# volser/FluidFramework

Measured on AMD Instinct MI355X. Metric: sequenced merge-tree ops applied/sec (whole node) + achieved HBM GB/s, higher is better.
Workload: dtype int32; 1 GPU; config2: 4096 docs x 8 clients x 10k msgs, lag U[0,32], 60/40 ins/rem; docs_per_gpu=4096, msgs_per_doc=10000, clients=8, lag_max=32, parallelism=doc-sharded x1, residency=blk, big_min_ops=0

## Files before the change

fluidframework_amd/csrc/mt_core.h:

```cpp
#pragma once
#include <type_traits>
#include "wave.h"
#include "../../include/mtgpu.h"

#define MT_MAXH 16
#define MT_PSK 16
#define MT_PKEYS MT_MAX_PROP_KEYS
#define MT_MAXN 8
#define MT_GRAN 256
#define MT_ZMAX 2
#define MT_NOREM 0x7FFFFFFF
#define MT_RFL 128
#ifndef MT_L_ROWS
#define MT_L_ROWS 256
#endif
#ifndef MT_L_BLKS
#define MT_L_BLKS 96
#endif
#ifndef MT_L_HEAP
#define MT_L_HEAP 96
#endif
#define MT_L_H 8
#ifndef MT_B_BLKS
#define MT_B_BLKS 104
// ... 220 lines not shown
#define MT_DREC_SLACK (2 + 2 * 2 * (8 + 64))

struct __attribute__((aligned(16))) MtLoadSeg {
    uint8_t flags, pad0; uint16_t client;
    int32_t seq, rseq;
    uint16_t rclient; int16_t prop;
    uint32_t poff, plen;
    uint32_t mid, pad1;
};
enum { MT_LD_START = 0, MT_LD_CONT = 1, MT_LD_REFLUSH = 2, MT_LD_REFLUSH_NEW = 3, MT_LD_UNSUPPORTED = 4 };
struct MtLoadStep { int seg, kind, cli, seq; };
struct MtLoad {
    const uint32_t* docs; const uint32_t* seg_off; const uint32_t* nhdr;
    const int32_t* ms; const int32_t* cs;
    const MtLoadSeg* segs; const uint16_t* payload;
    const uint32_t* plan_off; const MtLoadStep* plan;
};
#define MT_NONCOLLAB 0xFFFE
#define MT_NOBODY 0xFFFF

struct MtGen {
    unsigned long long seed;
    uint32_t ops, clients, lag_max, pct_insert, pct_remove, ins_len_max, rem_len_max, n_ann_sets, pct_rewrite;
    int enabled;
    const uint32_t* clients_per_run;
    uint32_t doc_id_base;
    uint32_t ins_len_min, seg_prop_sets, ins_at_end;
    uint64_t total_ops;
};

struct __attribute__((aligned(16))) MtQ16 { uint32_t x, y, z, w; };
struct __attribute__((aligned(16))) MtLdsPools {
    MtRow rows[MT_L_ROWS];
    MtBlk blk[MT_L_BLKS];
    MtHeapE heap[MT_L_HEAP + 2];
    int win[MT_L_ROWS];
    int uid[MT_L_ROWS];
    int udelta[MT_L_ROWS];
    uint8_t uanc[MT_L_ROWS * MT_L_H];
};

template <int NB, int NH, int NT, int NW> struct __attribute__((aligned(16))) MtLdsBlkT {
    static_assert(NB <= NT, "block ids index the corrections table");
    MtBlk blk[NB];
    MtHeapE heap[NH + 2];
    int win[NW];
    int bcorr[NT];
};
using MtLdsBlk = MtLdsBlkT<MT_B_BLKS, MT_B_HEAP, MT_B_BT, MT_B_W>;
using MtLdsBlkW = MtLdsBlkT<MT_BW_BLKS, MT_BW_HEAP, MT_BW_BT, MT_BW_W>;

struct __attribute__((aligned(16))) MtLdsBig {
    MtHeapE heap[MT_G_HEAP + 2];
    int win[MT_G_WIN];
    int uid[MT_G_U], udelta[MT_G_U];
    int uanc[MT_G_U * MT_G_H];
    uint16_t ulist[MT_G_U];
    MtBlk spare0; int spare1;
    int sid[MT_G_STG], sdel[MT_G_STG], spf[MT_G_STG];
    int htk[MT_G_HT], htv[MT_G_HT];
    uint16_t hlist[MT_G_HT];
    uint32_t bpc[MT_G_BP];
    struct Job {
        int op, r, c, r0, n, H, minSeq, heapN;
        MtRow* R; int* win; MtBlk* blk; int* uanc; uint16_t* text;
    } mw[2];
    int posted;
};

struct MtScratch {
    int pathB[MT_MAXH + 2], pathJ[MT_MAXH + 2];
    int pathOff[MT_MAXH + 2], pathLen[MT_MAXH + 2];
    int hold[64];
    int holdLen[64];
    uint8_t holdBlk[64];
    int rfree[MT_RFL];
    int corr[MT_MAXN];
};

struct __attribute__((aligned(16), may_alias)) MtQ16a { uint32_t x, y, z, w; };
#ifndef MT_RANGE_LEAF
#define MT_RANGE_LEAF 1
#endif
#ifndef MT_GT_CH
#define MT_GT_CH 4
#endif
MT_INLINE int pick16(const int* c, int j) {
    int v = c[0];
#pragma unroll
    for (int i = 1; i < 16; i++) v = (j == i) ? c[i] : v;
    return v;
}
MT_INLINE int pick8(const int* c, int j) {
    int v = c[0];
#pragma unroll
    for (int i = 1; i < 8; i++) v = (j == i) ? c[i] : v;
    return v;
}
MT_INLINE bool ovl_has(const MtOvx* ox, int n, unsigned long long ovl, int s, int rseq, int c) {
    if (c < 63) return ((ovl >> c) & 1ull) != 0;
    const bool more = (ovl >> 63) != 0;
    bool f = false;
    for (int i = 0; i < n; i++) {
        const MtOvx e = ox[i];
        f = f | (more & (e.row == s) & (e.client == c) & (e.rseq == rseq));
    }
    return f;
}
MT_INLINE bool vis_rc(int seq, uint32_t meta, int rseq, uint32_t rcl, unsigned long long ovl, int r, int c,
                      const MtOvx* ox, int nox, int s) {
    const int cl = (int)(meta & MT_M_CLIENT);
    const bool seen = (cl == c) | (seq <= r);
    const bool removed = (meta & MT_M_REMOVED) != 0;
    const bool gone = ((int)rcl == c) | (rseq <= r) | ovl_has(ox, nox, ovl, s, rseq, c);
    return seen & !(removed & gone);
}

struct BlkH { int len, parent, n, height, scour; };
struct ChildL { int len; bool tie; };
struct WinI { int id; int delta; int parent; bool live; bool recycle; };

enum { MT_WALK_SPLIT = 0, MT_WALK_INSERT = 1, MT_WALK_RANGE = 2 };
enum { MT_W_OK = 0, MT_W_NOCHANGE = 1, MT_W_FAIL = 2, MT_W_RANGED = 3 };
enum { MT_MAP_REMOVE = 0, MT_MAP_ANNOTATE = 1, MT_MAP_COLLECT = 2 };
enum { MT_PM_SET = 0, MT_PM_REWRITE = 1, MT_PM_INCR = 2, MT_PM_KEEP = 3, MT_PM_CONS = 4, MT_PM_INCR_SMIN = 5 };
MT_INLINE int mt_prop_mode(uint32_t fl) {
    if (!(fl & MT_OPF_COMBINE)) return (fl & MT_OPF_REWRITE) ? MT_PM_REWRITE : MT_PM_SET;
    if (fl & MT_OPF_REWRITE) return (fl & MT_OPF_CONSENSUS) ? MT_PM_CONS : MT_PM_KEEP;
    return (fl & MT_OPF_INCR_STRMIN) ? MT_PM_INCR_SMIN : MT_PM_INCR;
}

struct MtEngParams {
    uint32_t rowCap, heapCap, winCap, textCap, psetCap, p_nsets;
    uint16_t* textBase;
    const uint32_t* p_off; const uint16_t* p_key; const int32_t* p_val;
    const uint8_t* p_falsy; const uint32_t* p_class; const int32_t* p_vinfo;
};
#if defined(__HIP_DEVICE_COMPILE__)
#define MT_LDS_VAR(T, v) __shared__ T v
#else
#define MT_LDS_VAR(T, v) static T v
#endif
MT_LDS_VAR(MtLdsPools, mt_lds_pools_v);
MT_INLINE MtLdsPools& mt_lds() { return mt_lds_pools_v; }
MT_LDS_VAR(MtLdsBlk, mt_ldsb_v);
MT_INLINE MtLdsBlk& mt_ldsb() { return mt_ldsb_v; }
MT_LDS_VAR(MtLdsBlkW, mt_ldsbw_v);
MT_INLINE MtLdsBlkW& mt_ldsbw() { return mt_ldsbw_v; }
MT_LDS_VAR(MtLdsBig, mt_ldsg_v);
MT_INLINE MtLdsBig& mt_ldsg() { return mt_ldsg_v; }

struct MtCold {
    MtEngParams S;
    uint32_t cnt[6];
    int hw[2];
    int lcap[3];
    uint32_t gcap[4];
    int epoch, ncol, midcap;
    uint32_t op;
    MtDocHdr* hdr; int* rfhbm; MtOvx* ovx; int* midt; MtReg* regs;
    MtBlk* blk; MtHeapE* heap; int *uid, *udelta, *uanc; MtPSet* pset;
    int ovxn, blkfreen, texthalf, psettop;
    uint16_t* dtext; unsigned long long dtcap;
    uint32_t dused, tused; int dstop;
    int* regr; int regTop, regHalf, regCap;
    int pcKey[4], pcVal[4];
// ... 31 lines not shown
    MT_HD MtBlk& bk(int b) const {
        if constexpr (LDS) return mt_lds().blk[b]; else if constexpr (BLKL) return LB().blk[b];
        else return blk[b];
    }
    MT_HD MtHeapE& hp(int k) const {
        if constexpr (LDS) return mt_lds().heap[k]; else if constexpr (BLKL) return LB().heap[k];
        else if constexpr (BIG) return mt_ldsg().heap[k]; else return heap[k];
    }
    static constexpr int kW = BW ? MT_BW_W : MT_B_W;
    MT_HD int winGet(int k) const {
        if constexpr (BLKR) { if (k < kW) return LB().win[k]; return win[k]; }
        else return wn(k);
    }
    MT_HD void winSet(int k, int v) const {
        if constexpr (BLKR) { if (k < kW) LB().win[k] = v; else win[k] = v; }
        else wn(k) = v;
    }
    MT_HD int& wn(int k) const {
        static_assert(!BLKR, "block residency: winGet / winSet");
        if constexpr (LDS) return mt_lds().win[k];
        else if constexpr (BIG) { if (k < lRows) return mt_ldsg().win[k]; return win[k]; }
        else return win[k];
    }
    MT_HD int& ui(int k) const { if constexpr (LDS) return mt_lds().uid[k]; else return uid[k]; }
    MT_HD int& ud(int k) const { if constexpr (LDS) return mt_lds().udelta[k]; else return udelta[k]; }
    static constexpr bool UL = RES == MT_RES_BIG;
    static constexpr bool BT = BLKR;
    static constexpr int UCAP = RES == MT_RES_BIG ? MT_G_U : 0;
    template <bool L> MT_HD int uiAt(int k) const {
        if constexpr (UL && L) return mt_ldsg().uid[k];
        else return ui(k);
    }
    template <bool L> MT_HD int udAt(int k) const {
        if constexpr (UL && L) return mt_ldsg().udelta[k];
        else return ud(k);
    }
    template <bool L> MT_HD void uPutAt(int k, int id, int delta) {
        if constexpr (UL && L) { mt_ldsg().uid[k] = id; mt_ldsg().udelta[k] = delta; }
        else { ui(k) = id; ud(k) = delta; }
    }
    template <bool L> MT_HD void ancPutAt(int u, int h, int a) {
        if constexpr (UL && L) {
            static_assert(BIG, "block residency keeps per-block corrections, not ancestor chains");
            mt_ldsg().uanc[u * MT_G_H + h] = a;
        } else ancPut(u, h, a);
    }
    template <bool L> MT_HD int ancGetAt(int u, int h) const {
        if constexpr (UL && L) {
            static_assert(BIG, "block residency keeps per-block corrections, not ancestor chains");
            return mt_ldsg().uanc[u * MT_G_H + h];
        } else return ancGet(u, h);
    }
    MT_HD void ancPutAny(int u, int h, int a) {
        if constexpr (UL) { if (u < UCAP) ancPutAt<true>(u, h, a); else ancPutAt<false>(u, h, a); }
        else ancPut(u, h, a);
    }
    MT_HD int ancGetAny(int u, int h) const {
        if constexpr (UL) { if (u < UCAP) return ancGetAt<true>(u, h); return ancGetAt<false>(u, h); }
        else return ancGet(u, h);
    }
    template <class F> MT_HD void forU(F f) const {
        for (int base = 0; base < nU; base += MT_WAVE) {
            const int m = (nU - base) < MT_WAVE ? (nU - base) : MT_WAVE;
            if (UL && base < UCAP) f(std::true_type{}, base, m);
            else f(std::false_type{}, base, m);
        }
    }
    int root, height, minSeq, curSeq, rowTop, blkTop, blkFree, heapN, winN, textTop;
    int& psetTop = mt_cold_v.psettop;
    uint32_t status;
    uint32_t &c_ops = mt_cold_v.cnt[0], &c_msgs = mt_cold_v.cnt[1], &c_ins = mt_cold_v.cnt[2], &c_rows = mt_cold_v.cnt[3],
             &c_depth = mt_cold_v.cnt[4], &c_scour = mt_cold_v.cnt[5];
    unsigned long long prof[8];
    int& textHalf = mt_cold_v.texthalf; uint32_t blkCap;
    int nU; bool uValid; int uRef, uCli;
    int heapTop;
    int& gcEpoch = mt_cold_v.epoch;
    int lastL, lastIdx; bool lastSplit;
    bool htOk; int hlistN;
    bool htOn, pfOn; int mwSeq;
    bool bpOn;
    int& nCol = mt_cold_v.ncol;
    int landB;
    int rfN; int*& rfHbm = mt_cold_v.rfhbm;
    int& blkFreeN = mt_cold_v.blkfreen;
    int &heapHW = mt_cold_v.hw[0], &winHW = mt_cold_v.hw[1];
    static constexpr bool kLds = BLKL || BIG;
    int &lRows = mt_cold_v.lcap[0], &lBlks = mt_cold_v.lcap[1], &lHeap = mt_cold_v.lcap[2];
    uint32_t &gRowCap = mt_cold_v.gcap[0], &gBlkCap = mt_cold_v.gcap[1], &gHeapCap = mt_cold_v.gcap[2],
             &gWinCap = mt_cold_v.gcap[3];

    MT_HD void bind(const MtState& st, uint32_t d, MtScratch* scratch) {
        const MtDocLayout* Ly = st.layout + d;
        auto off = [&](const unsigned long long* p) -> size_t {
            const uint32_t* w = (const uint32_t*)p;
            return (size_t)uni(w[0]) | ((size_t)uni(w[1]) << 32);
        };
        S.rowCap = uni(Ly->rowCap); S.heapCap = uni(Ly->heapCap); S.winCap = uni(Ly->winCap); S.textCap = uni(Ly->textCap);
        S.psetCap = uni(Ly->psetCap); S.p_nsets = st.p_nsets; S.p_off = st.p_off; S.p_key = st.p_key; S.p_val = st.p_val;
        S.p_falsy = st.p_falsy; S.p_class = st.p_class; S.p_vinfo = st.p_vinfo; S.textBase = st.text + off(&Ly->text);
        blkCap = uni(Ly->blkCap); hdrp = st.hdr + d;
        R = st.rows + off(&Ly->row);
        blk = st.blk + off(&Ly->blk); heap = st.heap + off(&Ly->heap);
        const size_t wo = off(&Ly->win);
        win = st.win + wo; uid = st.uid + wo; udelta = st.udelta + wo; uanc = st.uanc + off(&Ly->anc);
        pset = st.pset + off(&Ly->pset);
        ovx = st.ovx + (size_t)d * MT_OVX_CAP;
        regs = st.reg + (size_t)d * MT_REG_CAP;
        regr = st.regr + off(&Ly->regr); regCap = (int)uni(Ly->regCap);
        midt = st.mid + off(&Ly->mid); midCap = (int)uni(Ly->midCap);
        drec = nullptr; dcount = nullptr; dcap = 0; curOp = 0;
        dtext = nullptr; dtcap = 0; dUsed = 0; tUsed = 0; dStop = 0;
        sc = scratch;
        const MtDocHdr& h = *hdrp;
        root = uni(h.root); height = uni(h.height); minSeq = uni(h.minSeq); curSeq = uni(h.curSeq); rowTop = uni(h.rowTop);
        blkTop = uni(h.blkTop); blkFree = uni(h.blkFree); heapN = uni(h.heapN); winN = uni(h.winN); textTop = uni(h.textTop);
        psetTop = uni(h.psetTop); status = uni(h.status); textHalf = uni(h.textHalf);
        text = S.textBase + (size_t)textHalf * S.textCap;
#if MT_KEEP_PROF
        for (int i = 0; i < 8; i++) prof[i] = h.prof[i];
#endif
        c_ops = c_msgs = c_ins = c_rows = c_depth = c_scour = 0;
        nU = 0; uValid = false; uRef = -1; uCli = -1;
        heapTop = heapN > 0 ? uni(heap[1].maxSeq) : 0x7FFFFFFF;
        lastL = 0; lastIdx = 0; lastSplit = false; gcEpoch = 0; htOk = false; hlistN = 0; htOn = pfOn = false; mwSeq = 0; bpOn = false;
        for (int i = 0; i < 4; i++) mt_cold_v.pcKey[i] = -1;
        rfHbm = st.hold + (size_t)d * MT_RFL; rfN = uni(h.rfN); blkFreeN = uni(h.blkFreeN);
        heapHW = uni(h.heapHW); winHW = uni(h.winHW); ovxN = uni(h.ovxN);
        regTop = uni(h.regTop); regHalf = uni(h.regHalf) & 1; mt_cold_v.pNever = uni(h.pNever);
        if (regTop < 0 || regTop > regCap) regTop = 0;
        if (ovxN < 0 || ovxN > MT_OVX_CAP) ovxN = 0;
        lRows = lBlks = lHeap = 0; gRowCap = gBlkCap = gHeapCap = gWinCap = 0;
        if (rfN < 0 || rfN > MT_RFL) rfN = 0;
        { const int n = rfN; const int* src = rfHbm;
          for (int base = 0; base < n; base += MT_WAVE) {
              const int m = (n - base) < MT_WAVE ? (n - base) : MT_WAVE;
              wave_for(m, [&](int k) MT_LAM { sc->rfree[base + k] = src[base + k]; });
          } }
        wave_sync();
    }
    MT_HD void store(uint32_t) {
        MtDocHdr& h = *hdrp;
        h.root = root; h.height = height; h.minSeq = minSeq; h.curSeq = curSeq; h.rowTop = rowTop;
        h.blkTop = blkTop; h.blkFree = blkFree; h.heapN = heapN; h.winN = winN; h.textTop = textTop;
        h.psetTop = psetTop; h.status = status; h.textHalf = textHalf; h.rfN = rfN; h.blkFreeN = blkFreeN;
        h.heapHW = heapHW; h.winHW = winHW; h.ovxN = ovxN; h.regTop = regTop; h.regHalf = regHalf;
        h.pNever = mt_cold_v.pNever;
        { const int n = rfN; int* dst = rfHbm;
          for (int base = 0; base < n; base += MT_WAVE) {
              const int m = (n - base) < MT_WAVE ? (n - base) : MT_WAVE;
              wave_for(m, [&](int k) MT_LAM { dst[base + k] = sc->rfree[base + k]; });
          } }
#if MT_KEEP_PROF
        for (int i = 0; i < 8; i++) h.prof[i] = prof[i];
#endif
        h.cnt[0] += c_ops; h.cnt[1] += c_msgs; h.cnt[2] += c_ins; h.cnt[3] += c_rows; h.cnt[4] += c_depth;
        h.cnt[5] += c_scour;
    }
    MT_HD void open() {
        root = 0; height = 0; minSeq = 0; curSeq = 0; rowTop = 0; blkTop = 1; blkFree = -1;
        heapN = 0; winN = 0; textTop = 0; psetTop = 0; status = 0; textHalf = 0; heapTop = 0x7FFFFFFF; rfN = 0;
        for (int i = 0; i < 4; i++) mt_cold_v.pcKey[i] = -1;
        blkFreeN = 0; heapHW = 0; winHW = 0; ovxN = 0;
        text = S.textBase;
        c_ops = c_msgs = c_ins = c_rows = c_depth = c_scour = 0;
        for (int i = 0; i < 6; i++) hdrp->cnt[i] = 0;
        for (int i = 0; i < 8; i++) prof[i] = 0;
#if !MT_KEEP_PROF
        for (int i = 0; i < 8; i++) hdrp->prof[i] = 0;
#endif
        wave_for(8, [&](int i) MT_LAM { bk(0).c[i] = -1; });
        bk(0).len = 0; bk(0).parent = -1; bk(0).n = 0; bk(0).height = 0; bk(0).scour = -1;
        bpReset();
        wave_for(MT_REG_CAP, [&](int i) MT_LAM { regs[i].client = -1; regs[i].n = 0; regs[i].flags = 0; regs[i].off = 0; });
        regTop = 0; regHalf = 0; mt_cold_v.pNever = 0;
    }

    MT_HD int allocRow() {
        if (rfN > 0) { rfN--; return uni(sc->rfree[rfN]); }
        if (rowTop >= (int)S.rowCap) { status |= MT_DS_OOM_ROWS; return -1; }
        return rowTop++;
    }
    MT_HD void freeRow(int s) { if (rfN < MT_RFL) { sc->rfree[rfN] = s; rfN++; } }
    MT_HD int allocBlock() {
        if (blkFree >= 0) { const int id = blkFree; blkFree = uni(bk(id).parent); blkFreeN--; return id; }
        if (blkTop >= (int)blkCap) { status |= MT_DS_OOM_BLOCKS; return -1; }
        return blkTop++;
    }
    MT_HD void freeBlock(int id) { bk(id).parent = blkFree; bk(id).n = -1; blkFree = id; blkFreeN++; bpDrop(id); }
    MT_HD static uint32_t bpPack(int b, int p) { return ((uint32_t)(b >> MT_G_BPL) << 20) | (uint32_t)(p + 1); }
    MT_HD void bpPut(int b, int p) {
        if constexpr (BIG) {
            if (bpOn) {
                uint32_t& e = mt_ldsg().bpc[b & (MT_G_BP - 1)];
                if (e != MT_BP_EMPTY && (e >> 20) != (uint32_t)(b >> MT_G_BPL)) MT_BS(4);
                e = bpPack(b, p);
            }
        }
    }
    MT_HD void bpDrop(int b) {
        if constexpr (BIG) {
            if (bpOn) {
                uint32_t& e = mt_ldsg().bpc[b & (MT_G_BP - 1)];
                if ((e >> 20) == (uint32_t)(b >> MT_G_BPL)) MT_BS(5);
                e = MT_BP_EMPTY;
            }
        }
    }
// ... 886 lines not shown
        int w = 0;
        for (int base = 0; base < n0; base += MT_WAVE) {
            const int m = (n0 - base) < MT_WAVE ? (n0 - base) : MT_WAVE;
            auto u = wave_map(m, [&](int k) MT_LAM { return lsN < 0 ? base + k : (int)mt_ldsg().ulist[base + k]; });
            auto keep = wave_map(m, [&](int k) MT_LAM { return mt_ldsg().uanc[own(u, k) * MT_G_H + hc] == child; });
            const auto rk = wave_rank(keep);
            const int cnt = wave_count(keep), w0 = w;
            wave_sync();
            wave_for(m, [&](int k) MT_LAM { if (own(keep, k)) mt_ldsg().ulist[w0 + own(rk, k)] = (uint16_t)own(u, k); });
            w += cnt;
        }
        wave_sync();
        return w;
    }

    MT_HD void ovxCompact() {
        int w = 0;
        for (int base = 0; base < ovxN; base += MT_WAVE) {
            const int m = (ovxN - base) < MT_WAVE ? (ovxN - base) : MT_WAVE;
            auto keep = wave_map(m, [&](int k) MT_LAM {
                const MtOvx e = ovx[base + k];
                return (bool)((int)(row(e.row).parent >= 0) & (int)(row(e.row).rseq == e.rseq) & (int)(e.rseq > minSeq));
            });
            auto ent = wave_map(m, [&](int k) MT_LAM { return ovx[base + k]; });
            auto rk = wave_rank(keep);
            const int cnt = wave_count(keep);
            wave_sync();
            const int w0 = w;
            wave_for(m, [&](int k) MT_LAM { if (own(keep, k)) ovx[w0 + own(rk, k)] = own(ent, k); });
            wave_sync();
            w += cnt;
        }
        ovxN = w;
    }
    MT_HD void ovxAdd(int s, int rseq, int c) {
        if (ovxN >= MT_OVX_CAP) ovxCompact();
        if (ovxN >= MT_OVX_CAP) { status |= MT_DS_OOM_OVERLAP; return; }
        MtOvx e; e.row = s; e.rseq = rseq; e.client = c; e.pad = 0;
        wave_for(1, [&](int) MT_LAM { ovx[ovxN] = e; });
        ovxN++;
    }
    MT_HD void ovxCopy(int s, int n) {
        const int rs = uni(row(s).rseq), n0 = ovxN;
        for (int base = 0; base < n0; base += MT_WAVE) {
            const int m = (n0 - base) < MT_WAVE ? (n0 - base) : MT_WAVE;
            auto hit = wave_map(m, [&](int k) MT_LAM { const MtOvx e = ovx[base + k]; return e.row == s && e.rseq == rs; });
            auto cl = wave_map(m, [&](int k) MT_LAM { return ovx[base + k].client; });
            uint64_t b = wave_ballot(hit);
            while (b) {
                const int k = __builtin_ctzll(b); b &= b - 1;
                ovxAdd(n, rs, wave_at(cl, k));
            }
        }
    }

    MT_HD static int rowDword(const MtRow& f, int k) {
        switch (k) {
            case 0: return f.len; case 1: return f.seq; case 2: return f.rseq; case 3: return (int)f.meta;
            case 4: return f.toff; case 5: return f.props; case 6: return f.parent; case 7: return f.tcap;
            case 8: return (int)(uint32_t)f.ovl; case 9: return (int)(uint32_t)(f.ovl >> 32);
            case 10: return (int)f.rcl; default: return f.mid;
        }
    }
    MT_HD static LaneArr<int> leafField(const LaneArr<MtRow>& lf, int k) {
        return wave_map(MT_WAVE, [&](int t) MT_LAM { return rowDword(own(lf, t), k); });
    }
    MT_HD int splitRow(int s, int pos, const LaneArr<MtRow>& lf, int j) {
        MT_EV2(5, 1);
        const int n = allocRow();
        if (n < 0) return -1;
        const uint32_t mt = (uint32_t)wave_at(leafField(lf, 3), j);
        const uint32_t ovh = (uint32_t)wave_at(leafField(lf, 9), j);
        wave_for(MT_WAVE, [&](int t) MT_LAM {
            if (t != j) return;
            MtRow q = own(lf, t);
            q.len -= pos; q.meta &= ~(MT_M_INWIN | MT_M_HREF); q.toff += pos; q.tcap -= pos; q.mid = 0;
            row(n) = q;
        });
        row(s).len = pos; row(s).tcap = pos;
        if (ovh >> 31) ovxCopy(s, n);
        if (mt & MT_M_INWIN) winAddKnown(n, mt & ~(MT_M_INWIN | MT_M_HREF));
        return n;
    }
    MT_HD void insertAtPath(int L, int idx, int node, int delta) {
        bool first = true;
        for (;;) {
            const int B = uni(sc->pathB[L]);
            BlkH h;
            auto cur = blkLoad(B, h);
            auto prv = wave_from8<-1>(cur);
            const int nd = node, ix = idx;
            auto nc = wave_map(8, [=](int i) MT_LAM {
                const int a = own(cur, i), b = own(prv, i);
                const int lt = -(int)(i < ix), eq = -(int)(i == ix);
                return (a & lt) | (nd & eq) | (b & ~(lt | eq));
            });
            const int n1 = h.n + 1;
            setChildParent(h.height, node, B);
            if (first) landB = B;
            if (n1 < MT_MAXN) {
                wave_for(8, [&](int i) MT_LAM { bk(B).c[i] = i < n1 ? own(nc, i) : -1; });
                bk(B).n = n1; bk(B).len = h.len + delta;
                if (delta != 0) wave_for(L, [&](int l) MT_LAM { const int pb = sc->pathB[l]; bk(pb).len = bk(pb).len + delta; });
                return;
            }
            lastSplit = true;
            MT_EV(6, 1);
            const int NB = allocBlock();
            if (NB < 0) return;
            auto hi = wave_from8<4>(nc);
            wave_for(8, [&](int i) MT_LAM {
                bk(NB).c[i] = i < 4 ? own(hi, i) : -1;
                bk(B).c[i] = i < 4 ? own(nc, i) : -1;
            });
            bk(NB).n = 4; bk(NB).height = h.height; bk(NB).scour = -1; bk(NB).parent = h.parent;
            bpPut(NB, h.parent);
            bk(B).n = 4;
            wave_for(4, [&](int i) MT_LAM { setChildParent(h.height, own(hi, i), NB); });
            if (first && ix >= 4) landB = NB;
            first = false;
            wave_sync();
            const int nbLen = sumObs(NB, 4, h.height), bLen = sumObs(B, 4, h.height);
            bk(NB).len = nbLen; bk(B).len = bLen;
            if (L == 0) {
                const int R = allocBlock();
                if (R < 0) return;
                wave_for(8, [&](int i) MT_LAM { bk(R).c[i] = i == 0 ? B : (i == 1 ? NB : -1); });
                bk(R).n = 2; bk(R).height = h.height + 1; bk(R).parent = -1; bk(R).scour = -1; bk(R).len = bLen + nbLen;
                bk(B).parent = R; bk(NB).parent = R;
                bpPut(R, -1); bpPut(B, R); bpPut(NB, R);
                root = R; height = h.height + 1;
                return;
            }
            node = NB; idx = uni(sc->pathJ[L - 1]) + 1; L = L - 1;
        }
    }
    MT_HD bool rangeLeaf(int B, int L, const BlkH& h, const LaneArr<int>& ch, const LaneArr<MtRow>& lf,
                         const LaneArr<ChildL>& cl, const LaneArr<int>& pre, int total, int p, int j, int span, int mode,
                         int c, int sq, int opset, int pm) {
        const int n = h.n, pe = p + span;
        if (span <= 0 || pe > total) return false;
        MT_EVR(2, 1);
        if (c >= 63 || mode > MT_MAP_ANNOTATE || (FULL && drec != nullptr)) { MT_EVR(4, 1); return false; }
        const auto len = wave_map(n, [&](int i) MT_LAM { return own(cl, i).len; });
        const auto meta = wave_map(n, [&](int i) MT_LAM { return own(lf, i).meta; });
        const auto ce = wave_map(n, [&](int i) MT_LAM {
            const int q = pe - own(pre, i), l = own(len, i);
            return (bool)((int)(q < l) | ((int)(q == 0) & (int)(l == 0) & (int)own(cl, i).tie));
        });
        const int je = wave_first(ce);
        const int pj = p - wave_at(pre, j), pje = je >= 0 ? pe - wave_at(pre, je) : 0;
        const uint32_t mj = wave_at(meta, j), mje = je >= 0 ? wave_at(meta, je) : 0u;
        const int s1 = (int)(pj > 0) & (int)!(mj & MT_M_MARKER), s2 = (int)(pje > 0) & (int)!(mje & MT_M_MARKER);
        const int ns = s1 + s2;
        if (n + ns >= MT_MAXN) { MT_EVR(3, 1); return false; }
        const auto cov = wave_map(n, [&](int i) MT_LAM {
            const int q = own(pre, i), l = own(len, i);
            return (bool)((int)(l > 0) & (int)(pe - q > 0) & (int)(p - q < l));
        });
        const bool rem = mode == MT_MAP_REMOVE;
        const auto add = wave_map(n, [&](int i) MT_LAM {
            return (bool)((int)own(cov, i) & (int)!(own(meta, i) & MT_M_INWIN) & (int)rem);
        });
        const bool side = wave_ballot(wave_map(n, [&](int i) MT_LAM {
            return (bool)((int)own(cov, i) & (int)(own(lf, i).ovl >> 63));
        })) != 0;
        const int w1 = s1 & (int)((mj & MT_M_INWIN) != 0), w2 = s2 & (int)((mje & MT_M_INWIN) != 0);
        const int nadd = wave_count(add);
        if (side || rfN + ((int)S.rowCap - rowTop) < ns || winN + w1 + w2 + nadd > (int)S.winCap) {
            MT_EVR(4, 1);
            return false;
        }
        MT_EVR(1, 1); MT_EVR(5, ns); MT_EV2(5, ns); MT_EV2(7, 1);
        int n1 = -1, n2 = -1;
        if (s1) n1 = allocRow();
        if (s2) n2 = allocRow();
        const int nact = wave_count(cov), first = wave_first(cov);
        const unsigned long long cbit = 1ull << c;
        const auto nd = wave_map(n, [&](int i) MT_LAM {
            const MtRow f = own(lf, i);
            const int isS = (int)(i == j) & s1, isE = (int)(i == je) & s2, isC = (int)own(cov, i);
            if (isE) {
                MtQ16a* d = (MtQ16a*)&row(n2);
                d[0] = MtQ16a{(uint32_t)(f.len - pje), (uint32_t)f.seq, (uint32_t)f.rseq, f.meta & ~MT_M_HREF};
                d[1] = MtQ16a{(uint32_t)(f.toff + pje), (uint32_t)f.props, (uint32_t)B, (uint32_t)(f.tcap - pje)};
                d[2] = MtQ16a{(uint32_t)f.ovl, (uint32_t)(f.ovl >> 32), f.rcl, 0u};
            }
            const int lo = isS ? pj : 0, hi = isE ? pje : f.len;
            if (isS) {
                ((MtQ16a*)&row(n1))[1] =
                    MtQ16a{(uint32_t)(f.toff + pj), (uint32_t)f.props, (uint32_t)B, (uint32_t)((isE ? pje : f.tcap) - pj)};
            }
            if (isS | isE) row(own(ch, i)).tcap = isS ? pj : pje;
            const int gone = (int)((f.meta & MT_M_REMOVED) != 0);
            const int mark = isC & (int)rem, fresh = mark & (gone ^ 1);
            const uint32_t crs = fresh ? (uint32_t)sq : (uint32_t)f.rseq, crc = fresh ? (uint32_t)c : f.rcl;
            const unsigned long long cov_ovl = (mark & gone) ? f.ovl | cbit : f.ovl;
            const uint32_t cm = mark ? f.meta | MT_M_REMOVED | MT_M_INWIN : f.meta;
            const int here = isC & (isS ^ 1);
            MtQ16a* own_ = (MtQ16a*)&row(own(ch, i));
            if (isS | isE | (here & mark))
                own_[0] = MtQ16a{(uint32_t)(isS ? pj : hi), (uint32_t)f.seq, here ? crs : (uint32_t)f.rseq, here ? cm : f.meta};
            if (here & mark) own_[2] = MtQ16a{(uint32_t)cov_ovl, (uint32_t)(cov_ovl >> 32), crc, (uint32_t)f.mid};
            if (isS) {
                MtQ16a* d = (MtQ16a*)&row(n1);
                d[0] = MtQ16a{(uint32_t)(hi - pj), (uint32_t)f.seq, crs, cm & ~MT_M_HREF};
                d[2] = MtQ16a{(uint32_t)cov_ovl, (uint32_t)(cov_ovl >> 32), crc, 0u};
            }
            return fresh ? hi - lo : 0;
        });
        const int obsDelta = -wave_sum8(nd);
        if (mode == MT_MAP_ANNOTATE) {
            const auto old = wave_map(n, [&](int i) MT_LAM { return own(lf, i).props; });
            const auto pid = wave_map(n, [&](int i) MT_LAM { return ((int)(i == j) & s1) ? n1 : own(ch, i); });
            int lastOld = -2, lastNew = -1;
            for (uint64_t b = wave_ballot(cov); b; b &= b - 1) {
                const int i = __builtin_ctzll(b), o = wave_at(old, i);
                if (o != lastOld) { lastNew = applyPropSet(o, opset, pm, sq); lastOld = o; }
                row(wave_at(pid, i)).props = lastNew;
            }
        }
        if (w1) winSet(winN++, n1);
        if (w2) winSet(winN++, n2);
        if (nadd) {
            const auto rk = wave_rank(add);
            const int w0 = winN;
            wave_for(n, [&](int i) MT_LAM {
                if (own(add, i)) winSet(w0 + own(rk, i), ((int)(i == j) & s1) ? n1 : own(ch, i));
            });
            winN += nadd;
        }
        if (winN > winHW) winHW = winN;
        if (ns) {
            wave_for(n, [&](int i) MT_LAM { bk(B).c[i + (s1 & (int)(i > j)) + (s2 & (int)(i > je))] = own(ch, i); });
            if (s1) bk(B).c[j + 1] = n1;
            if (s2) bk(B).c[je + 1 + s1] = n2;
            bk(B).n = n + ns;
            landB = B;
        }
        if (rem) {
            bk(B).len = h.len + obsDelta;
            if (L > 0 && obsDelta != 0) {
                wave_for(L, [&](int l) MT_LAM { const int pb = sc->pathB[l]; bk(pb).len = bk(pb).len + obsDelta; });
                wave_sync();
            }
        }
        if (first >= 0) {
            const bool half = first == j && s1;
            const uint32_t m0 = half ? mj & ~MT_M_HREF : wave_at(meta, first);
            addToLRUSetKnown(half ? n1 : wave_at(ch, first), sq, B, rem ? m0 | MT_M_REMOVED | MT_M_INWIN : m0);
        }
        c_rows += 2u * (uint32_t)(ns + nact);
        lastL = L; lastSplit = false; uValid = false;
        lastIdx = je < 0 ? n + s1 : (s2 ? je + 1 + s1 : je + (s1 & (int)(je > j)));
        return true;
    }
    MT_HD int walk(int kind, int pos, int r, int c, int cand, int candLen, int L0 = 0, int rEnd = 0, int rMode = 0,
                   int rSq = 0, int rOpset = -1, int rPm = 0) {
        if (!(uValid && uRef == r && uCli == c)) { computeU(r, c, false); L0 = 0; }
        int B = root, L = 0, p = pos;
        if (L0 > 0) { B = uni(sc->pathB[L0]); L = L0; p = pos - uni(sc->pathOff[L0]); }
        const bool narrow = BIG && nU <= UCAP && !htOk;
        int lsN = -1;
        BlkH h;
        MT_QB(q0); MT_QC(2);
        auto ch = blkLoad(B, h);
        MT_QE(0, q0);
        for (;;) {
            MT_EV(5, 1);
            sc->pathB[L] = B;
            MT_QB(q1);
            const bool kpre = !BLKL && h.height > 0;
            LaneArr<int> r0{}, r1{};
            if (kpre) kidsLoad(ch, h.n, r0, r1);
            LaneArr<MtRow> lf{};
            LaneArr<ChildL> cl;
            if (h.height == 0) {
                const int rr = r, cc = c;
                lf = wave_map(h.n, [&](int j) MT_LAM { return row(own(ch, j)); });
                cl = wave_map(h.n, [&](int j) MT_LAM {
                    const MtRow f = own(lf, j);
                    ChildL o;
                    o.len = vis_rc(f.seq, f.meta, f.rseq, f.rcl, f.ovl, rr, cc, ovx, ovxN, own(ch, j)) ? f.len : 0;
                    o.tie = !((f.meta & MT_M_REMOVED) && f.rseq <= rr);
                    return o;
                });
            } else cl = kpre ? childLens(B, h, ch, r, c, true, kidsLen(r0, r1), lsN) : childLens(B, h, ch, r, c);
            MT_QE(1, q1);
            auto lens = wave_map(h.n, [&](int j) MT_LAM { return own(cl, j).len; });
            auto pre = wave_excl_scan8(lens);
            const int total = wave_sum8(lens);
            sc->pathOff[L] = pos - p; sc->pathLen[L] = total;
            const bool interior = h.height > 0;
            auto cond = wave_map(h.n, [&](int j) MT_LAM {
                const int pj = p - own(pre, j), lj = own(cl, j).len;
                if (interior) return pj <= lj;
                return pj < lj || (pj == lj && pj == 0 && own(cl, j).tie);
            });
            const int j = wave_first(cond);
            if (j >= 0) {
                const int pj = p - wave_at(pre, j);
                if (interior) {
                    sc->pathJ[L] = j; L++; B = wave_at(ch, j); p = pj;
                    if (narrow && h.height > 1) lsN = narrowU(lsN, h.height - 1, B);
                    if (kpre) ch = kidRec(r0, r1, j, h); else ch = blkLoad(B, h);
                    continue;
                }
                const int s = wave_at(ch, j);
                lastL = L; lastSplit = false;
                if (MT_RANGE_LEAF && kind == MT_WALK_RANGE) {
                    if (rangeLeaf(B, L, h, ch, lf, cl, pre, total, p, j, rEnd - pos, rMode, c, rSq, rOpset, rPm))
                        return MT_W_RANGED;
                }
                if (kind != MT_WALK_INSERT) {
                    const uint32_t sm = (uint32_t)wave_at(leafField(lf, 3), j);
                    if (pj > 0 && !(sm & MT_M_MARKER)) {
                        const int n = splitRow(s, pj, lf, j);
                        if (n < 0) return MT_W_FAIL;
                        insertAtPath(L, j + 1, n, 0);
                        if (FULL && drec) {
                            const int ps = obsPosition(s);
                            const bool rm = (uni(row(s).meta) & MT_M_REMOVED) != 0;
                            emitDelta(MT_DK_SPLIT, ps, pj, s, n, uni(row(n).len));
                            (void)rm;
                        }
                        lastIdx = j + 1;
                        if (lastSplit) uValid = false;
                        return MT_W_OK;
                    }
                    lastIdx = j;
                    return MT_W_NOCHANGE;
                }
                insertAtPath(L, j, cand, candLen);
                uValid = false;
                return MT_W_OK;
            }
            if (p - total == 0) {
                lastL = L; lastIdx = h.n; lastSplit = false;
                if (kind != MT_WALK_INSERT) return MT_W_NOCHANGE;
                insertAtPath(L, h.n, cand, candLen);
                uValid = false;
                return MT_W_OK;
            }
            return MT_W_FAIL;
        }
    }

    MT_HD void heapAdd(int s, int ms) {
        if (heapN + 1 > (int)S.heapCap) { status |= MT_DS_OOM_HEAP; return; }
        int k = ++heapN;
        if (heapN > heapHW) heapHW = heapN;
        if (heapN < MT_WAVE) {
            const int n = heapN, dn = 31 - __builtin_clz((unsigned)n);
            auto mv = wave_map(n + 1, [&](int c) MT_LAM {
                c = mt_opaque(c);
                const int dc = 31 - __builtin_clz((unsigned)(c | 1));
                return (bool)((int)(c >= 2) & (int)((n >> (dn - dc)) == c));
            });
            auto pms = wave_map(n + 1, [&](int c) MT_LAM { return own(mv, c) ? (int)hp(mt_opaque(c) >> 1).maxSeq : 0; });
            auto psg = wave_map(n + 1, [&](int c) MT_LAM { return own(mv, c) ? (int)hp(mt_opaque(c) >> 1).seg : 0; });
            mv = wave_map(n + 1, [&](int c) MT_LAM { return own(mv, c) && own(pms, c) > ms; });
            const int top = wave_first(mv);
            k = top < 0 ? n : top >> 1;
            wave_for(n + 1, [&](int c) MT_LAM {
                if (own(mv, c)) { hp(c).seg = own(psg, c); hp(c).maxSeq = own(pms, c); }
                if (c == k) { hp(c).seg = s; hp(c).maxSeq = ms; }
            });
            if (k == 1) heapTop = ms;
            return;
        }
        while (k > 1) {
            const int pm = uni(hp(k >> 1).maxSeq);
            if (pm > ms) { hp(k).seg = hp(k >> 1).seg; hp(k).maxSeq = pm; k >>= 1; } else break;
        }
        hp(k).seg = s; hp(k).maxSeq = ms;
        if (k == 1) heapTop = ms;
    }
    MT_HD MtHeapE heapGet() {
        MT_EV(3, 1); MT_EV(7, heapN - 1);
        if (heapN < MT_WAVE) {
            const int N = heapN, n = N - 1;
            MtHeapE x; x.seg = uni(hp(1).seg); x.maxSeq = uni(hp(1).maxSeq);
            const int lseg = uni(hp(N).seg), lms = uni(hp(N).maxSeq);
            heapN = n;
            heapTop = 0x7FFFFFFF;
            if (n >= 1) {
                auto lm = wave_map(n + 1, [&](int i) MT_LAM { return (int)(i >= 1) & (int)(2 * i <= n) ? (int)hp(2 * mt_opaque(i)).maxSeq : 0; });
                auto rm = wave_map(n + 1, [&](int i) MT_LAM { return (int)(i >= 1) & (int)(2 * i < n) ? (int)hp(2 * mt_opaque(i) + 1).maxSeq : 0; });
                auto ls = wave_map(n + 1, [&](int i) MT_LAM { return (int)(i >= 1) & (int)(2 * i <= n) ? (int)hp(2 * mt_opaque(i)).seg : 0; });
                auto rs = wave_map(n + 1, [&](int i) MT_LAM { return (int)(i >= 1) & (int)(2 * i < n) ? (int)hp(2 * mt_opaque(i) + 1).seg : 0; });
                auto right = wave_map(n + 1, [&](int i) MT_LAM { return (bool)((int)(2 * i < n) & (int)(own(lm, i) > own(rm, i))); });
                auto cm = wave_map(n + 1, [&](int i) MT_LAM { return own(right, i) ? own(rm, i) : own(lm, i); });
                auto cs = wave_map(n + 1, [&](int i) MT_LAM { return own(right, i) ? own(rs, i) : own(ls, i); });
                auto nx = wave_map(n + 1, [&](int i) MT_LAM {
                    return (int)(i >= 1) & (int)(2 * i <= n) & (int)(own(cm, i) < lms) ? 2 * i + (int)own(right, i) : 0;
                });
                int k = 1;
                for (int t = wave_at(nx, 1); t != 0; t = wave_at(nx, t)) { MT_EV(4, 1); k = t; }
                const int dk = 31 - __builtin_clz((unsigned)k);
                wave_for(n + 1, [&](int i) MT_LAM {
                    if (i < 1 || i > k) return;
// ... 838 lines not shown
            const int w0 = winN;
            wave_for(m, [&](int k) MT_LAM {
                if (own(inw, k)) { const int s = base + k; winSet(w0 + own(rk, k), s); row(s).meta = row(s).meta | MT_M_INWIN; }
            });
            winN += cnt;
        }
        if (winN > winHW) winHW = winN;
        blkTop = 0; blkFree = -1; blkFreeN = 0;
        bpReset();
        int first = 0, count = nh, h = 0;
        for (;;) {
            const int nb = (count + MT_MAXN - 2) / (MT_MAXN - 1);
            if (blkTop + nb > (int)blkCap) { status |= MT_DS_OOM_BLOCKS; return; }
            const int b0 = blkTop; blkTop += nb;
            const int lvl = h, f0 = first, cnt = count;
            for (int base = 0; base < nb; base += MT_WAVE) {
                const int m = (nb - base) < MT_WAVE ? (nb - base) : MT_WAVE;
                wave_for(m, [&](int k) MT_LAM {
                    const int B = b0 + base + k, c0 = (base + k) * (MT_MAXN - 1);
                    const int n = (cnt - c0) < (MT_MAXN - 1) ? (cnt - c0) : (MT_MAXN - 1);
                    int len = 0;
                    for (int i = 0; i < MT_MAXN; i++) {
                        const int id = i < n ? f0 + c0 + i : -1;
                        if (id >= 0) {
                            if (lvl == 0) { row(id).parent = B; len += (row(id).meta & MT_M_REMOVED) ? 0 : row(id).len; }
                            else { bk(id).parent = B; len += bk(id).len; }
                        }
                        bk(B).c[i] = id;
                    }
                    bk(B).n = n; bk(B).len = len; bk(B).height = lvl; bk(B).parent = -1; bk(B).scour = -1;
                });
            }
            wave_sync();
            if (nb == 1) { root = b0; height = lvl; return; }
            first = b0; count = nb; h++;
        }
    }
    MT_HD int loadInsert(const MtLoad& Ld, uint32_t gi, int pos, int cli, int sq, bool boundary) {
        if (boundary) { walk(MT_WALK_SPLIT, pos, 0, cli, -1, 0); if (status) return 0; }
        const MtLoadSeg* g = Ld.segs + gi;
        const uint32_t fl = uni((uint32_t)g->flags);
        const bool mk = (fl & MT_LS_MARKER) != 0, rm = (fl & MT_LS_REMOVED) != 0;
        const int plen = mk ? 0 : uni((int)g->plen);
        const int L = mk ? 1 : plen;
        if (L == 0) return 0;
        const int n = allocRow();
        if (n < 0) return 0;
        row(n).len = L; row(n).seq = sq; row(n).rseq = rm ? uni(g->rseq) : MT_NOREM;
        row(n).meta = (uint32_t)cli | (rm ? MT_M_REMOVED : 0u) | (mk ? MT_M_MARKER : 0u);
        row(n).rcl = rm ? (uint32_t)uni((int)g->rclient) : 0u;
        row(n).ovl = 0ull; row(n).parent = -1; row(n).props = -1;
        {
            const int mi = mk ? uni((int)g->mid) : 0;
            row(n).mid = mi;
            if (mi) { if (mi > midCap) { status |= MT_DS_UNSUPPORTED; return 0; } midt[mi - 1] = n; }
        }
        row(n).tcap = plen;
        if (mk) row(n).toff = uni((int)g->plen);
        else {
            const int t0 = textAlloc(plen);
            if (t0 < 0) return 0;
            row(n).toff = t0;
            const uint16_t* src = Ld.payload + uni((int)g->poff);
            for (int base = 0; base < plen; base += MT_WAVE) {
                const int m = (plen - base) < MT_WAVE ? (plen - base) : MT_WAVE;
                wave_for(m, [&](int k) MT_LAM { text[t0 + base + k] = src[base + k]; });
            }
            c_ins += (uint64_t)plen;
        }
        const int pid = uni((int)g->prop);
        if (pid >= 0) { const int ps = newPropMap(pid); row(n).props = ps; }
        wave_sync();
        if (status) return 0;
        const int w = walk(MT_WALK_INSERT, pos, 0, cli, n, rm ? 0 : L);
        if (w != MT_W_OK || uni(row(n).parent) < 0) { status |= MT_DS_INSERT_FAILED; return 0; }
        c_rows += 2;
        if (sq > minSeq || rm) winAdd(n);
        if (sq > minSeq) addToLRUSet(n, sq);
        return L;
    }
    MT_HD void opInsert(int pos, int r, int c, int sq, const uint16_t* src, int plen, bool marker, int refType, int segProps,
                        int markerId, const LaneArr<int>& pay) {
        MT_PB(t0);
        int w = walk(MT_WALK_SPLIT, pos, r, c, -1, 0);
        MT_PE(MT_PH_SPLIT, t0);
        if (w == MT_W_OK) c_rows += 2;
        if (status) return;
        const int L = marker ? 1 : plen;
        if (L > 0) {
            const int n = allocRow();
            if (n < 0) return;
            const bool nonl = !marker && plen <= MT_WAVE &&
                              wave_count(wave_map(plen, [&](int k) MT_LAM { return own(pay, k) == (int)'\n'; })) == 0;
            const uint32_t m0 = (uint32_t)c | (marker ? MT_M_MARKER : 0u) | (nonl ? MT_M_NONL : 0u);
            row(n).len = L; row(n).seq = sq; row(n).rseq = MT_NOREM;
            row(n).meta = m0;
            row(n).ovl = 0ull; row(n).parent = -1; row(n).rcl = 0u;
            row(n).mid = markerId >= 0 ? markerId + 1 : 0;
            if (markerId >= 0) {
                if (markerId >= midCap) { status |= MT_DS_UNSUPPORTED; return; }
                midt[markerId] = n;
            }
            row(n).props = segProps >= 0 ? newPropMap(segProps) : -1;
            row(n).tcap = marker ? 0 : plen;
            if (marker) row(n).toff = refType;
            else {
                row(n).parent = -1;
                const int t0 = textAlloc(plen);
                if (t0 < 0) return;
                row(n).toff = t0;
                if (plen <= MT_WAVE) wave_for(plen, [&](int k) MT_LAM { text[t0 + k] = (uint16_t)own(pay, k); });
                else {
                    for (int base = 0; base < plen; base += MT_WAVE) {
                        const int m = (plen - base) < MT_WAVE ? (plen - base) : MT_WAVE;
                        wave_for(m, [&](int k) MT_LAM { text[t0 + base + k] = src[base + k]; });
                    }
                }
                c_ins += (uint64_t)plen;
            }
            wave_sync();
            MT_PB(t1);
            landB = -1;
            if ((w == MT_W_OK || w == MT_W_NOCHANGE) && !lastSplit) {
                insertAtPath(lastL, lastIdx, n, L);
                uValid = false;
                w = MT_W_OK;
            } else {
                w = walk(MT_WALK_INSERT, pos, r, c, n, L);
            }
            MT_PE(MT_PH_INSERT, t1);
            if (w != MT_W_OK || landB < 0) { status |= MT_DS_INSERT_FAILED; return; }
            c_rows += 2;
            const uint32_t m1 = winAddKnown(n, m0);
            if (sq > minSeq) addToLRUSetKnown(n, sq, landB, m1);
            if (FULL && drec) emitDelta(MT_DK_INSERT, obsPosition(n), L, n, uni(row(n).props), -1, -1);
        }
        zamboni();
    }
    MT_HD int regFind(int c, int name, bool alloc) {
        auto cl = wave_map(MT_REG_CAP, [&](int i) MT_LAM { return regs[i].client; });
        auto nm = wave_map(MT_REG_CAP, [&](int i) MT_LAM { return regs[i].name; });
        const int hit = wave_first(wave_map(MT_REG_CAP, [&](int i) MT_LAM { return own(cl, i) == c && own(nm, i) == name; }));
        if (hit >= 0 || !alloc) return hit;
        return wave_first(wave_map(MT_REG_CAP, [&](int i) MT_LAM { return own(cl, i) < 0; }));
    }
    MT_HD void opCopy(int start, int end, int r, int c, int name) {
        const int e = regFind(c, name, true);
        if (e < 0) { status |= MT_DS_UNSUPPORTED; return; }
        nCol = 0;
        const uint32_t cr0 = c_rows;
        rangeMap(MT_MAP_COLLECT, start, end, r, c, 0, -1, MT_PM_SET);
        if (status) return;
        if (regTop + nCol > regCap) {
            regCompact();
            if (regTop + nCol > regCap) { status |= MT_DS_UNSUPPORTED; return; }
            nCol = 0; c_rows = cr0;
            rangeMap(MT_MAP_COLLECT, start, end, r, c, 0, -1, MT_PM_SET);
            if (status) return;
        }
        const int n = nCol, base = regTop;
        if (n > rfN + ((int)S.rowCap - rowTop)) { status |= MT_DS_OOM_ROWS; return; }
        const int f0 = rfN, t0 = rowTop;
        uint64_t rem = 0;
        for (int b0 = 0; b0 < n; b0 += MT_WAVE) {
            const int m = (n - b0) < MT_WAVE ? (n - b0) : MT_WAVE;
            const auto rm = wave_map(m, [&](int k) MT_LAM {
                const int i = b0 + k, s = regRow(base + i);
                const int d = i < f0 ? sc->rfree[f0 - 1 - i] : t0 + (i - f0);
                const uint32_t mt = row(s).meta;
                row(d).len = row(s).len; row(d).seq = row(s).seq; row(d).rseq = row(s).rseq;
                row(d).meta = (mt & (MT_M_CLIENT | MT_M_REMOVED | MT_M_MARKER | MT_M_NONL)) | MT_M_REG;
                row(d).rcl = row(s).rcl; row(d).props = row(s).props; row(d).mid = row(s).mid;
                row(d).toff = row(s).toff; row(d).tcap = (mt & MT_M_MARKER) ? 0 : row(s).len;
                row(d).ovl = 0ull; row(d).parent = -1;
                regRow(base + i) = d;
                return (mt & MT_M_REMOVED) != 0;
            });
            rem |= wave_ballot(rm);
        }
        rfN = n < f0 ? f0 - n : 0;
        rowTop = t0 + (n > f0 ? n - f0 : 0);
        wave_sync();
        MtReg& g = regs[e];
        const int on = uni(g.client) == c ? uni(g.n) : 0, of = uni(g.flags), oo = uni(g.off);
        if (on > 0 && !(of & 2)) {
            for (int i = 0; i < on; i++) {
                const int s = uni(regRow(oo + i));
                row(s).meta = uni(row(s).meta) & ~MT_M_REG;
                freeRow(s);
            }
        }
        const int fl = rem ? 1 : 0;
        wave_for(1, [&](int) MT_LAM { g.client = c; g.name = name; g.n = n; g.flags = fl; g.off = base; });
        regTop = base + n;
        wave_sync();
    }
    MT_HD void regCompact() {
        const auto ns = wave_map(MT_REG_CAP, [&](int i) MT_LAM { return regs[i].client >= 0 ? regs[i].n : 0; });
        const auto os = wave_map(MT_REG_CAP, [&](int i) MT_LAM { return regs[i].off; });
        const int other = regHalf ^ 1;
        int* dst = regr + (size_t)other * regCap;
        int w = 0;
        for (int e = 0; e < MT_REG_CAP; e++) {
            const int n = wave_at(ns, e), o = wave_at(os, e);
            if (n <= 0) continue;
            for (int b0 = 0; b0 < n; b0 += MT_WAVE) {
                const int m = (n - b0) < MT_WAVE ? (n - b0) : MT_WAVE;
                wave_for(m, [&](int k) MT_LAM { dst[w + b0 + k] = regRow(o + b0 + k); });
            }
            const int w0 = w;
            wave_for(1, [&](int) MT_LAM { regs[e].off = w0; });
            w += n;
        }
        wave_sync();
        regHalf = other; regTop = w;
    }
    MT_HD void opPaste(int pos, int r, int c, int sq, int name) {
        const int e = regFind(c, name, false);
// ... 91 lines not shown
```

Measured before the change: 277.4 million ops/s.

## Fuse split-row and new-row insertion into one leaf update on insert

On insert, the split half produced by walking to the position is no longer inserted into the leaf immediately. It is deferred and placed together with the new row in a single two-child insertAtPath pass, which saves one leaf rewrite and a possible extra block split. The block-split logic is generalised to handle nine children with an asymmetric 5/4 split. A leaf-split fallback for range removal is also added but stays off by default (MT_LEAF_SPLIT 0). This adds complexity and correctness risk in landB and LRU tracking.

Measured after the change: 283.7 million ops/s (median of 6 runs). +2.3%, better.

```diff
diff --git a/fluidframework_amd/csrc/mt_core.h b/fluidframework_amd/csrc/mt_core.h
--- a/fluidframework_amd/csrc/mt_core.h
+++ b/fluidframework_amd/csrc/mt_core.h
@@ -326,6 +326,12 @@
 #ifndef MT_RANGE_LEAF
 #define MT_RANGE_LEAF 1
 #endif
+#ifndef MT_LEAF_SPLIT
+#define MT_LEAF_SPLIT 0
+#endif
+#ifndef MT_INSERT_LEAF
+#define MT_INSERT_LEAF 1
+#endif
 #ifndef MT_GT_CH
 #define MT_GT_CH 4
 #endif
@@ -523,6 +529,7 @@
     bool bpOn;
     int& nCol = mt_cold_v.ncol;
     int landB;
+    int pendR;
     int rfN; int*& rfHbm = mt_cold_v.rfhbm;
     int& blkFreeN = mt_cold_v.blkfreen;
     int &heapHW = mt_cold_v.hw[0], &winHW = mt_cold_v.hw[1];
@@ -564,7 +571,7 @@
         c_ops = c_msgs = c_ins = c_rows = c_depth = c_scour = 0;
         nU = 0; uValid = false; uRef = -1; uCli = -1;
         heapTop = heapN > 0 ? uni(heap[1].maxSeq) : 0x7FFFFFFF;
-        lastL = 0; lastIdx = 0; lastSplit = false; gcEpoch = 0; htOk = false; hlistN = 0; htOn = pfOn = false; mwSeq = 0; bpOn = false;
+        lastL = 0; lastIdx = 0; lastSplit = false; pendR = -1; gcEpoch = 0; htOk = false; hlistN = 0; htOn = pfOn = false; mwSeq = 0; bpOn = false;
         for (int i = 0; i < 4; i++) mt_cold_v.pcKey[i] = -1;
         rfHbm = st.hold + (size_t)d * MT_RFL; rfN = uni(h.rfN); blkFreeN = uni(h.blkFreeN);
         heapHW = uni(h.heapHW); winHW = uni(h.winHW); ovxN = uni(h.ovxN);
@@ -1617,7 +1624,9 @@
         if (mt & MT_M_INWIN) winAddKnown(n, mt & ~(MT_M_INWIN | MT_M_HREF));
         return n;
     }
-    MT_HD void insertAtPath(int L, int idx, int node, int delta) {
+    template <bool PAIR = false>
+    MT_HD void insertAtPath(int L, int idx, int node, int delta, int half = -1, int hidx = 0, int late = 0, int watch = 0) {
+        if (!PAIR) watch = idx;
         bool first = true;
         for (;;) {
             const int B = uni(sc->pathB[L]);
@@ -1625,12 +1634,25 @@
             auto cur = blkLoad(B, h);
             auto prv = wave_from8<-1>(cur);
             const int nd = node, ix = idx;
-            auto nc = wave_map(8, [=](int i) MT_LAM {
-                const int a = own(cur, i), b = own(prv, i);
-                const int lt = -(int)(i < ix), eq = -(int)(i == ix);
-                return (a & lt) | (nd & eq) | (b & ~(lt | eq));
-            });
-            const int n1 = h.n + 1;
+            const bool two = PAIR && first && half >= 0;
+            LaneArr<int> nc;
+            if (two) {
+                auto prv2 = wave_from8<-2>(cur);
+                const int hf = half, hx = hidx;
+                nc = wave_map(9, [=](int i) MT_LAM {
+                    const int a = own(cur, i), b = own(prv, i), b2 = own(prv2, i);
+                    const int lt = -(int)(i < ix), eq = -(int)(i == ix), mid = -((int)(i > ix) & (int)(i < hx)),
+                              e2 = -(int)(i == hx);
+                    return (a & lt) | (nd & eq) | (b & mid) | (hf & e2) | (b2 & ~(lt | eq | mid | e2));
+                });
+            } else {
+                nc = wave_map(8, [=](int i) MT_LAM {
+                    const int a = own(cur, i), b = own(prv, i);
+                    const int lt = -(int)(i < ix), eq = -(int)(i == ix);
+                    return (a & lt) | (nd & eq) | (b & ~(lt | eq));
+                });
+            }
+            const int n1 = h.n + (two ? 2 : 1);
             setChildParent(h.height, node, B);
             if (first) landB = B;
             if (n1 < MT_MAXN) {
@@ -1643,19 +1665,20 @@
             MT_EV(6, 1);
             const int NB = allocBlock();
             if (NB < 0) return;
-            auto hi = wave_from8<4>(nc);
+            const int kb = (two && n1 == MT_MAXN + 1 && late <= 4) ? 5 : 4, kn = two ? n1 - kb : 4;
+            auto hi = kb == 5 ? wave_from8<5>(nc) : wave_from8<4>(nc);
             wave_for(8, [&](int i) MT_LAM {
-                bk(NB).c[i] = i < 4 ? own(hi, i) : -1;
-                bk(B).c[i] = i < 4 ? own(nc, i) : -1;
+                bk(NB).c[i] = i < kn ? own(hi, i) : -1;
+                bk(B).c[i] = i < kb ? own(nc, i) : -1;
             });
-            bk(NB).n = 4; bk(NB).height = h.height; bk(NB).scour = -1; bk(NB).parent = h.parent;
+            bk(NB).n = kn; bk(NB).height = h.height; bk(NB).scour = -1; bk(NB).parent = h.parent;
             bpPut(NB, h.parent);
-            bk(B).n = 4;
-            wave_for(4, [&](int i) MT_LAM { setChildParent(h.height, own(hi, i), NB); });
-            if (first && ix >= 4) landB = NB;
+            bk(B).n = kb;
+            wave_for(kn, [&](int i) MT_LAM { setChildParent(h.height, own(hi, i), NB); });
+            if (first && watch >= kb) landB = NB;
             first = false;
             wave_sync();
-            const int nbLen = sumObs(NB, 4, h.height), bLen = sumObs(B, 4, h.height);
+            const int nbLen = sumObs(NB, kn, h.height), bLen = sumObs(B, kb, h.height);
             bk(NB).len = nbLen; bk(B).len = bLen;
             if (L == 0) {
                 const int R = allocBlock();
@@ -1688,7 +1711,8 @@
         const uint32_t mj = wave_at(meta, j), mje = je >= 0 ? wave_at(meta, je) : 0u;
         const int s1 = (int)(pj > 0) & (int)!(mj & MT_M_MARKER), s2 = (int)(pje > 0) & (int)!(mje & MT_M_MARKER);
         const int ns = s1 + s2;
-        if (n + ns >= MT_MAXN) { MT_EVR(3, 1); return false; }
+        const bool room = n + ns < MT_MAXN;
+        if (!room) { MT_EVR(3, 1); if (!MT_LEAF_SPLIT) return false; }
         const auto cov = wave_map(n, [&](int i) MT_LAM {
             const int q = own(pre, i), l = own(len, i);
             return (bool)((int)(l > 0) & (int)(pe - q > 0) & (int)(p - q < l));
@@ -1702,11 +1726,13 @@
         })) != 0;
         const int w1 = s1 & (int)((mj & MT_M_INWIN) != 0), w2 = s2 & (int)((mje & MT_M_INWIN) != 0);
         const int nadd = wave_count(add);
-        if (side || rfN + ((int)S.rowCap - rowTop) < ns || winN + w1 + w2 + nadd > (int)S.winCap) {
-            MT_EVR(4, 1);
+        const bool blocks = room || blkFreeN + ((int)blkCap - blkTop) >= L + 2;
+        if (side || rfN + ((int)S.rowCap - rowTop) < ns || winN + w1 + w2 + nadd > (int)S.winCap || !blocks) {
+            if (room) { MT_EVR(4, 1); }
             return false;
         }
-        MT_EVR(1, 1); MT_EVR(5, ns); MT_EV2(5, ns); MT_EV2(7, 1);
+        if (room) { MT_EVR(1, 1); } else { MT_EVR(7, 1); }
+        MT_EVR(5, ns); MT_EV2(5, ns); MT_EV2(7, 1);
         int n1 = -1, n2 = -1;
         if (s1) n1 = allocRow();
         if (s2) n2 = allocRow();
@@ -1766,32 +1792,48 @@
             winN += nadd;
         }
         if (winN > winHW) winHW = winN;
-        if (ns) {
+        bool firstKept = true;
+        int first2 = -1;
+        if (!room) {
+            const int kb = (ns == 2 && n == MT_MAXN - 1 && je + 2 <= 4) ? 5 : 4;
+            const auto inNew = wave_map(n, [&](int i) MT_LAM {
+                const int f = ((int)(i == j) & s1) ? j + 1 : i + (s1 & (int)(i > j)) + (s2 & (int)(i > je));
+                return (bool)((int)own(cov, i) & (int)(f >= kb));
+            });
+            first2 = wave_first(inNew);
+            firstKept = first2 != first;
+            wave_sync();
+            if (ns == 2) insertAtPath<true>(L, j + 1, n1, obsDelta, n2, je + 2, je + 2, MT_MAXN);
+            else insertAtPath<true>(L, s1 ? j + 1 : je + 1, s1 ? n1 : n2, obsDelta, -1, 0, 0, MT_MAXN);
+            wave_sync();
+        } else if (ns) {
             wave_for(n, [&](int i) MT_LAM { bk(B).c[i + (s1 & (int)(i > j)) + (s2 & (int)(i > je))] = own(ch, i); });
             if (s1) bk(B).c[j + 1] = n1;
             if (s2) bk(B).c[je + 1 + s1] = n2;
             bk(B).n = n + ns;
             landB = B;
         }
-        if (rem) {
+        if (rem && room) {
             bk(B).len = h.len + obsDelta;
             if (L > 0 && obsDelta != 0) {
                 wave_for(L, [&](int l) MT_LAM { const int pb = sc->pathB[l]; bk(pb).len = bk(pb).len + obsDelta; });
                 wave_sync();
             }
         }
-        if (first >= 0) {
-            const bool half = first == j && s1;
-            const uint32_t m0 = half ? mj & ~MT_M_HREF : wave_at(meta, first);
-            addToLRUSetKnown(half ? n1 : wave_at(ch, first), sq, B, rem ? m0 | MT_M_REMOVED | MT_M_INWIN : m0);
-        }
+        auto lru = [&](int i, int blk) MT_LAM {
+            const bool half = i == j && s1;
+            const uint32_t m0 = half ? mj & ~MT_M_HREF : wave_at(meta, i);
+            addToLRUSetKnown(half ? n1 : wave_at(ch, i), sq, blk, rem ? m0 | MT_M_REMOVED | MT_M_INWIN : m0);
+        };
+        if (first >= 0 && firstKept) lru(first, B);
+        if (!room && first2 >= 0) lru(first2, landB);
         c_rows += 2u * (uint32_t)(ns + nact);
-        lastL = L; lastSplit = false; uValid = false;
+        lastL = L; lastSplit = !room; uValid = false;
         lastIdx = je < 0 ? n + s1 : (s2 ? je + 1 + s1 : je + (s1 & (int)(je > j)));
         return true;
     }
     MT_HD int walk(int kind, int pos, int r, int c, int cand, int candLen, int L0 = 0, int rEnd = 0, int rMode = 0,
-                   int rSq = 0, int rOpset = -1, int rPm = 0) {
+                   int rSq = 0, int rOpset = -1, int rPm = 0, bool defer = false) {
         if (!(uValid && uRef == r && uCli == c)) { computeU(r, c, false); L0 = 0; }
         int B = root, L = 0, p = pos;
         if (L0 > 0) { B = uni(sc->pathB[L0]); L = L0; p = pos - uni(sc->pathOff[L0]); }
@@ -1852,6 +1894,10 @@
                     if (pj > 0 && !(sm & MT_M_MARKER)) {
                         const int n = splitRow(s, pj, lf, j);
                         if (n < 0) return MT_W_FAIL;
+                        if (MT_INSERT_LEAF && kind == MT_WALK_SPLIT && defer) {
+                            pendR = n; lastIdx = j + 1;
+                            return MT_W_OK;
+                        }
                         insertAtPath(L, j + 1, n, 0);
                         if (FULL && drec) {
                             const int ps = obsPosition(s);
@@ -2856,7 +2902,9 @@
     MT_HD void opInsert(int pos, int r, int c, int sq, const uint16_t* src, int plen, bool marker, int refType, int segProps,
                         int markerId, const LaneArr<int>& pay) {
         MT_PB(t0);
-        int w = walk(MT_WALK_SPLIT, pos, r, c, -1, 0);
+        const bool pair = MT_INSERT_LEAF && !(FULL && drec != nullptr);
+        pendR = -1;
+        int w = walk(MT_WALK_SPLIT, pos, r, c, -1, 0, 0, 0, 0, 0, -1, 0, pair);
         MT_PE(MT_PH_SPLIT, t0);
         if (w == MT_W_OK) c_rows += 2;
         if (status) return;
@@ -2895,7 +2943,14 @@
             wave_sync();
             MT_PB(t1);
             landB = -1;
-            if ((w == MT_W_OK || w == MT_W_NOCHANGE) && !lastSplit) {
+            if (pair) {
+                if (w == MT_W_OK || w == MT_W_NOCHANGE) {
+                    insertAtPath<true>(lastL, lastIdx, n, L, pendR, lastIdx + 1, lastIdx, lastIdx);
+                    if (pendR >= 0) { MT_EVR(6, lastSplit ? (1ull << 32) + 1 : 1); }
+                    uValid = false;
+                    w = MT_W_OK;
+                }
+            } else if ((w == MT_W_OK || w == MT_W_NOCHANGE) && !lastSplit) {
                 insertAtPath(lastL, lastIdx, n, L);
                 uValid = false;
                 w = MT_W_OK;
@@ -2908,6 +2963,9 @@
             const uint32_t m1 = winAddKnown(n, m0);
             if (sq > minSeq) addToLRUSetKnown(n, sq, landB, m1);
             if (FULL && drec) emitDelta(MT_DK_INSERT, obsPosition(n), L, n, uni(row(n).props), -1, -1);
+        } else if (pendR >= 0) {
+            insertAtPath(lastL, lastIdx, pendR, 0);
+            if (lastSplit) uValid = false;
         }
         zamboni();
     }
```
